# NoSameRain/RayTracingRenderer

Measured on AMD Instinct MI355X. Metric: Mray/s (traced closest-hit + shadow rays) at 1024x1024x64spp, synthetic 1M triangles, higher is better.
Workload: dtype f32; 1 GPU; C3: synth-1M, 1024x1024, 64 spp, MAX_DEPTH 4; triangles=1000000, width=1024, height=1024, spp=64, chunk_spp=64, max_depth=4, parallelism=one GPU, every tile (no exchange)

## Files before the change

### raytracingrenderer_amd/build.py

```python
import os
import shutil
import subprocess
import tempfile
import sys

ROOT = os.path.dirname(os.path.dirname(os.path.abspath(__file__)))
PKG = os.path.join(ROOT, "raytracingrenderer_amd")
CSRC = os.path.join(PKG, "csrc")
LIB = os.path.join(PKG, "lib")
ORACLE = os.path.join(ROOT, "oracle")
ORACLE_BUILD = os.path.join(ORACLE, "_build")
HIPCC = os.environ.get("HIPCC", "/opt/rocm/bin/hipcc")
ARCH = os.environ.get("RTG_ARCH", "gfx950")

HOST_SRC = ["host/image_io.cpp", "host/jpeg_decode.cpp", "host/gem_json.cpp", "host/scene_front.cpp"]
DEVICE_SRC = ["device/rtg_trace.hip", "device/rtg_scene.hip", "device/rtg_render.hip", "device/rtg_api.hip",
              "device/rtg_shade.hip", "device/rtg_light.hip", "device/rtg_multi.hip", "device/rtg_bvh.hip",
              "device/rtg_denoise.hip", "device/rtg_env.hip", "device/rtg_light_pick.hip",
              "device/rtg_shade_phys.hip", "device/rtg_shade_mis.hip"]
DEVICE_FLAGS = {"device/rtg_shade.hip": ["-mllvm", "-amdgpu-sched-strategy=max-ilp", "-fno-slp-vectorize"]}
DEVICE_FLAGS.update({"device/rtg_%s.hip" % u: ["-fno-slp-vectorize"] for u in ("trace", "scene", "render", "api")})
DEVICE_FLAGS["device/rtg_light_pick.hip"] = DEVICE_FLAGS["device/rtg_shade.hip"]
DEVICE_FLAGS["device/rtg_shade_phys.hip"] = DEVICE_FLAGS["device/rtg_shade.hip"]
DEVICE_FLAGS["device/rtg_shade_mis.hip"] = DEVICE_FLAGS["device/rtg_shade.hip"]
# ... 94 lines not shown

def build_device(force=False, debug=False):
    d = os.path.join(LIB, "debug") if debug else LIB
    os.makedirs(d, exist_ok=True)
    out = os.path.join(d, "librtg.so")
    if force or _stale(out, "device", "rtg-build-id:", debug):
        _compile_and_link(out, source_hash("device", debug), ["-DRTG_DEBUG=1"] if debug else [])
    return out


def build_variant(name, extra_flags):
    os.makedirs(os.path.join(LIB, "ab"), exist_ok=True)
    return _compile_and_link(os.path.join(LIB, "ab", name + ".so"), "ab-" + name, extra_flags)


def build_cli(force=False):
    out = os.path.join(LIB, "rtg_render")
    src = [os.path.join(CSRC, "host", "cli.cpp")]
    if not os.path.exists(src[0]):
        return None
    if force or _newer(out, _deps(src) + [os.path.join(LIB, "librth.so")]):
        _run(["g++", "-std=c++17", "-O2", "-ffp-contract=off", "-o", out] + src +
             ["-L" + LIB, "-lrth", "-lrtg", "-Wl,-rpath,$ORIGIN", "-ldl"])
    return out


def build_oracle(force=False):
    os.makedirs(ORACLE_BUILD, exist_ok=True)
    src = os.path.join(ORACLE, "rt_oracle.c")
    outs = []
    for flavour, libm in (("rtm", "0"), ("libm", "1")):
        out = os.path.join(ORACLE_BUILD, "liboracle_%s.so" % flavour)
        if force or _newer(out, _deps([src])):
            _run(["gcc", "-std=c11", "-O2", "-ffp-contract=off", "-fPIC", "-shared", "-D_GNU_SOURCE",
                  "-DORACLE_LIBM=" + libm, "-o", out, src, "-lm", "-lpthread"])
        outs.append(out)
    chk = os.path.join(ORACLE_BUILD, "libm_check")
    chk_src = os.path.join(ORACLE, "libm_check.c")
    if force or _newer(chk, _deps([chk_src])):
        _run(["gcc", "-std=c11", "-O2", "-ffp-contract=off", "-fno-builtin", "-pthread", "-o", chk, chk_src, "-lm"])
    outs.append(chk)
    dv = os.path.join(ORACLE_BUILD, "div_rewrites")
    dv_src = os.path.join(ORACLE, "div_rewrites.c")
    if force or _newer(dv, [dv_src]):
        _run(["gcc", "-std=c11", "-O2", "-ffp-contract=off", "-D_GNU_SOURCE", "-pthread", "-o", dv, dv_src, "-lm"])
    outs.append(dv)
    return outs


SAN_FLAGS = ["-O1", "-g", "-fsanitize=address,undefined", "-fno-sanitize-recover=all", "-fno-omit-frame-pointer",
             "-ffp-contract=off"]


def build_sanitized(force=False):
    nat = os.path.join(ROOT, "tests", "native")
    out_dir = os.path.join(nat, "_build")
    os.makedirs(out_dir, exist_ok=True)
    out = os.path.join(out_dir, "host_sanitize")
    drv = os.path.join(nat, "host_sanitize.cpp")
    orc = os.path.join(ORACLE, "rt_oracle.c")
    src = [os.path.join(CSRC, s) for s in HOST_SRC]
    if force or _newer(out, _deps(src + [drv, orc])):
        obj = os.path.join(out_dir, "rt_oracle_san.o")
        _run(["gcc", "-std=c11", "-D_GNU_SOURCE", "-DORACLE_LIBM=0", "-c", "-o", obj, orc] + SAN_FLAGS)
        _run(["g++", "-std=c++17", "-o", out, drv] + src + [obj] + SAN_FLAGS + ["-lz", "-lpthread", "-lm"])
    return out


def _build_test_program(name, extra_src, libs, force):
    nat = os.path.join(ROOT, "tests", "native")
    os.makedirs(os.path.join(nat, "_build"), exist_ok=True)
    out = os.path.join(nat, "_build", name)
    src = [os.path.join(nat, name + ".cpp")] + extra_src
    if force or _newer(out, _deps(src) + [os.path.join(LIB, "lib%s.so" % l) for l in libs]):
        _run([HIPCC, "-O2", "-std=c++17", "-ffp-contract=off", "-o", out] + src +
             ["-L" + LIB] + ["-l" + l for l in libs] + ["-Wl,-rpath," + LIB])
    return out


def build_sbvh_check(force=False):
    return _build_test_program("sbvh_check", [os.path.join(CSRC, "device", "rtg_bvh.hip")], ["rth"], force)


def build_scene_digest(force=False):
    return _build_test_program("scene_digest", [], ["rth", "rtg"], force)


def build_ref(force=False):
    mk = os.path.join(ORACLE, "ref", "Makefile")
    if not os.path.isdir("/root/reference/RTBase") or not os.path.exists(mk):
        return None
    _run(["make", "-s", "-C", os.path.join(ORACLE, "ref")] + (["-B"] if force else []))
    return os.path.join(ORACLE, "_ref", "libref.so")


def stage_assets():
    src = "/root/reference/RTBase"
    dst = os.path.join(ROOT, "assets")
    if not os.path.isdir(src):
        return
    os.makedirs(dst, exist_ok=True)
    for name in ("coffee", "bathroom", "materialball"):
        if os.path.isdir(os.path.join(src, name)) and not os.path.isdir(os.path.join(dst, name)):
            shutil.copytree(os.path.join(src, name), os.path.join(dst, name))
    for f, into in (("GI.hdr", ""), ("GI.hdr", "coffee")):
        d = os.path.join(dst, into, f)
        if os.path.exists(os.path.join(src, f)) and os.path.isdir(os.path.dirname(d)) and not os.path.exists(d):
            shutil.copy(os.path.join(src, f), d)


def build_all(force=False, device=True):
    stage_assets()
    build_host(force)
    if device:
        build_device(force)
        build_device(force, debug=True)
    build_cli(force)
    build_oracle(force)
    build_ref(force)


if __name__ == "__main__":
    build_all(force="--force" in sys.argv, device="--no-device" not in sys.argv)
    print("ok")
```

### raytracingrenderer_amd/csrc/device/rtg_bvh.hip

```cpp
#include "rtg_internal.h"

#include <algorithm>
#include <array>
#include <atomic>
#include <cmath>
#include <cstring>
#include <thread>
#include <vector>

namespace {

struct Ref {
    int tri;
    double lo[3], hi[3];
};

struct Box {
    double lo[3] = {INFINITY, INFINITY, INFINITY}, hi[3] = {-INFINITY, -INFINITY, -INFINITY};
    void add(const double* l, const double* h) {
        for (int a = 0; a < 3; ++a) { lo[a] = std::min(lo[a], l[a]); hi[a] = std::max(hi[a], h[a]); }
    }
    void add(const Ref& r) { add(r.lo, r.hi); }
    void add(const Box& b) { add(b.lo, b.hi); }
    bool empty() const { return lo[0] > hi[0]; }
    double area() const {
        if (empty()) return 0.0;
        const double x = hi[0] - lo[0], y = hi[1] - lo[1], z = hi[2] - lo[2];
        return x * y + y * z + z * x;
    }
};

double overlap_area(const Box& a, const Box& b) {
    Box o;
    for (int k = 0; k < 3; ++k) {
        o.lo[k] = std::max(a.lo[k], b.lo[k]);
        o.hi[k] = std::min(a.hi[k], b.hi[k]);
        if (o.lo[k] > o.hi[k]) return 0.0;
    }
    return o.area();
}

bool clip_bounds(const double v[3][3], const double* lo, const double* hi, double* out_lo, double* out_hi) {
    double a[12][3], b[12][3];
    int n = 3;
    for (int i = 0; i < 3; ++i)
        for (int k = 0; k < 3; ++k) a[i][k] = v[i][k];
    for (int ax = 0; ax < 3; ++ax)
        for (int side = 0; side < 2; ++side) {
            const double c = side ? hi[ax] : lo[ax];
            auto inside = [&](const double* p) { return side ? p[ax] <= c : p[ax] >= c; };
            int m = 0;
            for (int i = 0; i < n; ++i) {
                const double* p = a[i];
                const double* q = a[(i + 1) % n];
                const bool pi = inside(p), qi = inside(q);
                if (pi) { std::memcpy(b[m++], p, sizeof(double) * 3); }
                if (pi != qi && m < 12) {
                    const double t = (c - p[ax]) / (q[ax] - p[ax]);
                    for (int k = 0; k < 3; ++k) b[m][k] = p[k] + t * (q[k] - p[k]);
                    b[m][ax] = c;
                    ++m;
                }
            }
            n = std::min(m, 9);
            if (n == 0) return false;
            std::memcpy(a, b, sizeof(double) * 3 * n);
        }
    for (int k = 0; k < 3; ++k) { out_lo[k] = INFINITY; out_hi[k] = -INFINITY; }
    for (int i = 0; i < n; ++i)
        for (int k = 0; k < 3; ++k) {
            out_lo[k] = std::min(out_lo[k], a[i][k]);
            out_hi[k] = std::max(out_hi[k], a[i][k]);
        }
    for (int k = 0; k < 3; ++k) {
        out_lo[k] = std::max(out_lo[k], lo[k]);
        out_hi[k] = std::min(out_hi[k], hi[k]);
        if (out_lo[k] > out_hi[k]) return false;
    }
    return true;
}

struct Builder {
    const rtg_scene_desc* d;
    std::vector<int32_t> lk;
    std::vector<Ref> leaf_ref;
    double root_area = 0.0;
    long budget = 0;
// ... 139 lines not shown
        double best = INFINITY;
        ax = -1;
        for (int a = 0; a < 3; ++a)
            if (cost[a] < best) { best = cost[a]; ax = a; plane = pl[a]; }
        return best;
    }

    int build(std::vector<Ref>& r, int depth) {
        const int node = new_node();
        if (!ok) return node;
        if (depth > 120) { ok = false; return node; }
        if (depth >= stop_depth && r.size() > 1) {
            deferred.emplace_back(node, std::move(r));
            return node;
        }
        if (r.size() == 1) {
            leaf_ref[node] = r[0];
            lk[(size_t)node * 4 + 2] = r[0].tri;
            lk[(size_t)node * 4 + 3] = r[0].tri + 1;
            return node;
        }
        Box nb, cb;
        for (const Ref& x : r) {
            nb.add(x);
            double c[3];
            for (int k = 0; k < 3; ++k) c[k] = 0.5 * (x.lo[k] + x.hi[k]);
            cb.add(c, c);
        }
        std::vector<int> order;
        size_t cut = 0;
        Box bl, br;
        const double co = object_split(r, cb, order, cut, bl, br);
        const bool have_o = !order.empty() && cut > 0 && cut < r.size();
        int sax = -1;
        double plane = 0.0;
        double cs = INFINITY;
        if (budget > 0 && (!have_o || overlap_area(bl, br) > RTG_SBVH_ALPHA * root_area))
            cs = spatial_split(r, nb, sax, plane);
        std::vector<Ref> L, R;
        if (sax >= 0 && cs < co) {
            long dup = 0;
            for (const Ref& x : r) {
                if (x.hi[sax] <= plane) { L.push_back(x); continue; }
                if (x.lo[sax] >= plane) { R.push_back(x); continue; }
                double v[3][3];
                tri(x.tri, v);
                Ref a = x, b = x;
                double sl[3], sh[3];
                for (int k = 0; k < 3; ++k) { sl[k] = x.lo[k]; sh[k] = x.hi[k]; }
                sh[sax] = plane;
                const bool ka = clip_bounds(v, sl, sh, a.lo, a.hi);
                for (int k = 0; k < 3; ++k) { sl[k] = x.lo[k]; sh[k] = x.hi[k]; }
                sl[sax] = plane;
                const bool kb = clip_bounds(v, sl, sh, b.lo, b.hi);
                if (ka) L.push_back(a);
                if (kb) R.push_back(b);
                if (!ka && !kb) L.push_back(x);
                if (ka && kb) ++dup;
            }
            if (L.empty() || R.empty() || (L.size() >= r.size() && R.size() >= r.size())) {
                L.clear();
                R.clear();
            } else {
                budget -= dup;
            }
        }
        if (L.empty()) {
            if (have_o) {
                for (size_t i = 0; i < order.size(); ++i) (i < cut ? L : R).push_back(r[order[i]]);
            } else {
                L.assign(r.begin(), r.begin() + r.size() / 2);
                R.assign(r.begin() + r.size() / 2, r.end());
            }
        }
        std::vector<Ref>().swap(r);
        const int l = build(L, depth + 1);
        const int rr = build(R, depth + 1);
        lk[(size_t)node * 4] = l;
        lk[(size_t)node * 4 + 1] = rr;
        return node;
    }
};

}

bool build_sbvh(const rtg_scene_desc* d, std::vector<int32_t>& lk, std::vector<float>& bd) {
    const uint32_t nt = d->n_tris;
    if (nt < 2) return false;
    for (size_t k = 0; k < (size_t)nt * 9; ++k)
        if (!std::isfinite(d->positions[k])) return false;
    float scale = 0.0f;
    for (int k = 0; k < 6; ++k)
        if (std::isfinite(d->node_bounds[k])) scale = std::max(scale, std::fabs(d->node_bounds[k]));
    const double eta = std::ldexp((double)scale, -17);
    std::vector<Ref> refs(nt);
    Box root;
    for (uint32_t t = 0; t < nt; ++t) {
        const float* P = d->positions + (size_t)t * 9;
        refs[t].tri = (int)t;
        for (int k = 0; k < 3; ++k) {
            refs[t].lo[k] = std::min(std::min((double)P[k], (double)P[3 + k]), (double)P[6 + k]);
            refs[t].hi[k] = std::max(std::max((double)P[k], (double)P[3 + k]), (double)P[6 + k]);
        }
        root.add(refs[t]);
    }
    const int threads = (int)std::max(1u, std::min(16u, std::thread::hardware_concurrency()));
    Builder top(d);
    top.root_area = root.area();
    top.budget = (long)((double)nt * RTG_SBVH_DUP);
    top.stop_depth = nt < 50000 || threads == 1 ? (1 << 30) : 6;
    top.build(refs, 0);
    if (!top.ok) return false;
    const size_t nsub = top.deferred.size();
    std::vector<Builder> sub;
    sub.reserve(nsub);
    long deferred_refs = 0;
    for (auto& dr : top.deferred) deferred_refs += (long)dr.second.size();
    for (size_t k = 0; k < nsub; ++k) {
        sub.emplace_back(d);
        sub[k].root_area = top.root_area;
        sub[k].budget = deferred_refs ? (long)((double)top.budget * (double)top.deferred[k].second.size() / deferred_refs) : 0;
    }
    {
        std::atomic<size_t> next{0};
        std::vector<std::thread> pool;
        for (int t = 0; t < std::min<int>(threads, (int)nsub); ++t)
            pool.emplace_back([&]() {
                for (size_t k; (k = next.fetch_add(1)) < nsub;) sub[k].build(top.deferred[k].second, 6);
            });
        for (auto& t : pool) t.join();
    }
    for (const Builder& b : sub)
        if (!b.ok) return false;
    std::vector<int32_t> L = std::move(top.lk);
    std::vector<Ref> R = std::move(top.leaf_ref);
    for (size_t k = 0; k < nsub; ++k) {
        const int ph = top.deferred[k].first;
        const int base = (int)R.size();
        auto id = [&](int j) { return j == 0 ? ph : base + j - 1; };
        const Builder& b = sub[k];
        for (size_t j = 0; j < b.leaf_ref.size(); ++j) {
            int32_t w[4] = {b.lk[j * 4], b.lk[j * 4 + 1], b.lk[j * 4 + 2], b.lk[j * 4 + 3]};
            if (w[0] >= 0) { w[0] = id(w[0]); w[1] = id(w[1]); }
            if (j == 0) {
                std::memcpy(&L[(size_t)ph * 4], w, sizeof(w));
                R[ph] = b.leaf_ref[0];
            } else {
                L.insert(L.end(), w, w + 4);
                R.push_back(b.leaf_ref[j]);
            }
        }
    }
    const size_t nn = R.size();
    bd.assign(nn * 6, 0.0f);
    for (size_t i = nn; i-- > 0;) {
        float* o = &bd[i * 6];
        const Ref& x = R[i];
        if (L[i * 4] < 0) {
            for (int k = 0; k < 3; ++k) {
                o[k] = std::nextafter((float)(x.lo[k] - eta), -INFINITY);
                o[3 + k] = std::nextafter((float)(x.hi[k] + eta), INFINITY);
            }
        } else {
            const float* a = &bd[(size_t)L[i * 4] * 6];
            const float* b = &bd[(size_t)L[i * 4 + 1] * 6];
            for (int k = 0; k < 3; ++k) {
                o[k] = std::min(a[k], b[k]);
                o[3 + k] = std::max(a[3 + k], b[3 + k]);
            }
        }
    }
    lk = std::move(L);
    return true;
}
```

### raytracingrenderer_amd/csrc/device/rtg_internal.h

```cpp
#pragma once
#include "rtg_dev.h"
#include "../../../include/rtg.h"
#include "rtg_phys.h"
#include "rtg_mis.h"

#include <hip/hip_runtime.h>
#include <rocprofiler-sdk-roctx/roctx.h>

#include <string>
#include <vector>

using namespace rtgd;

#define RTG_TB 256
#define RTG_NSTATS 24
#ifndef RTG_TTB
#define RTG_TTB 64
#endif
#define RTG_POP ((int)0x80000001)
#ifndef RTG_STACK
#define RTG_STACK 16
#endif
#ifndef RTG_STACK_SMALL
#define RTG_STACK_SMALL 7
#endif
#ifndef RTG_SMALL_F4
#define RTG_SMALL_F4 192
#endif
#ifndef RTG_POSTPONE
#define RTG_POSTPONE 32
#endif
#ifndef RTG_MEM_PCT
#define RTG_MEM_PCT 50
#endif
#ifndef RTG_REFILL
#define RTG_REFILL 12
#endif
#ifndef RTG_TRACE_WPE
#define RTG_TRACE_WPE 7
#endif
#define RTG_CULL_REL 1.52587890625e-05f
#ifndef RTG_FETCH
#define RTG_FETCH 256
#endif
#ifndef RTG_FETCH_TAIL
#define RTG_FETCH_TAIL 8
#endif
#ifndef RTG_TAIL_BATCH
#define RTG_TAIL_BATCH 64
#endif
#ifndef RTG_LDS_MATS
#define RTG_LDS_MATS 64
#endif
#ifndef RTG_LDS_LIGHTS
#define RTG_LDS_LIGHTS 48
#endif
#ifndef RTG_LDS_PHYS
#define RTG_LDS_PHYS 64
#endif
#ifndef RTG_SHADE_WAVES
#define RTG_SHADE_WAVES 7
#endif
#ifndef RTG_SHADE_ENV_ALT_WAVES
#define RTG_SHADE_ENV_ALT_WAVES 4
#endif
#ifndef RTG_SAH_SWEEP
#define RTG_SAH_SWEEP 2048
#endif
#ifndef RTG_SAH_BINS
#define RTG_SAH_BINS 128
#endif
#ifndef RTG_SBVH_BINS
#define RTG_SBVH_BINS 32
#endif
#ifndef RTG_SBVH_ALPHA
#define RTG_SBVH_ALPHA 1e-5
#endif
#ifndef RTG_SBVH_DUP
#define RTG_SBVH_DUP 0.5
#endif
#define RTG_CAP_LEN 64
#ifndef RTG_DEBUG
#define RTG_DEBUG 0
#endif
#define RTG_CAM_PER_SAMPLE 1
#define RTG_CAM_LENS 2

#define RTG_CPAD(f) unsigned f; unsigned f##_pad[31];
struct __align__(16) Counters {
    RTG_CPAD(n_ext) RTG_CPAD(n_shadow) RTG_CPAD(f_ext) RTG_CPAD(f_shadow) RTG_CPAD(f_shade)
    RTG_CPAD(n_cam)
    RTG_CPAD(pad1) RTG_CPAD(pad2)
    unsigned f8[8 * 32];
    unsigned ne8[8 * 32];
    unsigned ns8[8 * 32];
};
#undef RTG_CPAD
static inline size_t seg_tiles(size_t P) { return ((P + 255) / 256 + 7) / 8; }
static inline size_t queue_slots(size_t P) { return seg_tiles(P) * 8 * 256; }

struct TraceIO {
    const unsigned* queue;
    const float4* ray_o;
    const float4* ray_d;
    const unsigned* count;
    float4* hits;
    const unsigned* squeue;
    const float4* sray_o;
    const float4* sray_d;
    const float4* sray_c;
    int spos;
    const unsigned* scount;
    float4* contrib;
    int* visible;
    unsigned* fetch;
    unsigned* fetch8;
    unsigned seg_cap;
    const unsigned* seg_ne;
    const unsigned* seg_ns;
    int* ovf;
    unsigned long long* stats;
    int cull;
    int wide;
    unsigned long long* wtime;
    uint4* cap;
    unsigned* cap_len;
    unsigned cap_n;
    float4 cam_o;
    unsigned* hcnt;
};

struct ChunkArgs {
    const unsigned* pixlist;
    unsigned npix, ns, s0, P;
    unsigned long long seed;
    int max_depth;
    int mode;
    DevCamera cam;
    int lean = 0;
    unsigned seg_tiles = 0;
    int cam_mode = 0;
    unsigned long long ns_mul = 0;
    unsigned ns_shift = 0;
};
static inline void set_ns_div(ChunkArgs& a) {
    a.ns_mul = 0;
    if ((unsigned long long)a.P > (1ull << 31)) return;
    unsigned l = 0;
    while ((1u << l) < a.ns) ++l;
    const unsigned S = 31 + l;
    a.ns_mul = ((1ull << S) + a.ns - 1) / a.ns;
    a.ns_shift = S;
}
static __device__ __forceinline__ void split_pid(const ChunkArgs& a, unsigned pid, unsigned& lp, unsigned& sl) {
    lp = a.ns_mul ? (unsigned)(((unsigned long long)pid * a.ns_mul) >> a.ns_shift) : pid / a.ns;
    sl = pid - lp * a.ns;
}

struct PathBufs {
    float4* thr;
    unsigned long long* rng;
    float4* ray_o;
// ... 121 lines not shown
    unsigned next_slot = 0;
    hipEvent_t entry = nullptr;
    hipEvent_t last_fold = nullptr;
    bool inflight = false;
    uint32_t pend_first = 0, pend_n = 0;
    uint64_t pend_seed = 0;
    std::vector<uint32_t> pend_key;
    int no_coalesce = 0;
    unsigned* d_pix = nullptr;
    size_t cap_pix = 0;
    std::vector<uint32_t> pix_key;
    unsigned npix = 0;
    unsigned* d_qctr = nullptr;
    unsigned long long* d_stats = nullptr;
    rtg_stats stats{};
    hipEvent_t ev[4] = {nullptr, nullptr, nullptr, nullptr};
    std::vector<hipEvent_t> kev;
    unsigned* h_cnt = nullptr;
    unsigned* d_hcnt = nullptr;
    int cap_cnt = 0;
    std::vector<hipEvent_t> tev;
    DenoiseState* dn = nullptr;
    int env_mode = RTG_ENV_UNIFORM;
    bool env_light = false;
    bool env_built = false;
    uint4* d_env_table = nullptr;
    std::vector<uint32_t> env_entries;
    std::vector<double> env_weights;
    double env_build_ms = 0.0;
    rtg_light_sampling light_sampling{RTG_LIGHTS_UNIFORM, 0.125f};
    bool light_built = false;
    float light_built_share = 0.0f;
    uint4* d_light_table = nullptr;
    std::vector<uint32_t> light_entries;
    std::vector<double> light_weights;
    double light_build_ms = 0.0;
    int material_model = RTG_MATERIALS_REFERENCE;
    std::vector<uint32_t> tri_mat;
    uint32_t n_desc_mats = 0;
    std::vector<rtg_material_params> mat_params;
    bool phys_built = false;
    bool phys_any = false;
    PhysMat* d_phys = nullptr;
    unsigned* d_phys_index = nullptr;
    int n_phys = 0;
    std::vector<unsigned> phys_index;
    int path_mis = RTG_PATH_MIS_OFF;
    std::vector<int32_t> light_tri;
    std::vector<int32_t> light_of;
    uint2* d_mis_index = nullptr;
    PhysMat* d_mis_ref = nullptr;
    int n_mis_ref = 0;
};
#define RTG_CNT_PENDING 0xFFFFFFFFu

struct HostScene {
    std::vector<DevNode> nodes;
    std::vector<DevNodeQ> nodesq;
    std::vector<float4> leafbox;
    std::vector<float4> img;
    int img_tri = 0, img_lb = 0;
    std::vector<DevTri48> tris48;
    std::vector<DevShade> shade;
    std::vector<DevMat> mats;
    std::vector<DevLight> lights;
    std::vector<DevTex> texinfo;
    std::vector<float> texels;
    int n_lights = 0, env_tex = -1, env_off = 0, env_w = 1, env_h = 1;
    bool env_uniform = false;
    float env_one[3] = {0.0f, 0.0f, 0.0f};
    int root_word = RTG_EXIT, root_wordw = RTG_EXIT;
    bool usew = false, rebuilt = false;
    uint32_t bvh_depth = 0, wide_depth = 0;
    float root_box[6] = {0, 0, 0, 0, 0, 0};
    float cull_scale = 0.0f;
    DevCamera cam{};
    rtg_camera_proj proj{};
    std::vector<uint32_t> tri_mat;
    uint32_t n_desc_mats = 0;
    std::vector<int32_t> light_tri;
};

bool build_sbvh(const rtg_scene_desc* d, std::vector<int32_t>& lk, std::vector<float>& bd);
int prepare_scene(const rtg_scene_desc* d, HostScene& hs);
int upload_scene(int device, const HostScene& hs, rtg_handle* h);
int size_trace_grids(rtg_handle* h);
static inline int trace_blocks_max(const rtg_handle* h) {
    return std::max({h->trace_blocks[0][0], h->trace_blocks[0][1], h->trace_blocks[1][0], h->trace_blocks[1][1]});
}
int capture_begin(rtg_handle* h, TraceIO& io, unsigned seg_tiles, hipStream_t ss);
int launch_trace(rtg_handle* h, const TraceIO& io, hipStream_t st, unsigned max_blocks = 0);
void free_chunk(ChunkSlot& sl);
int ensure_ovf(rtg_handle* h, ChunkSlot& sl);
int set_pixels(rtg_handle* h, const uint32_t* tiles, uint32_t n_tiles);
int ensure_chunk(rtg_handle* h, ChunkSlot& sl, size_t P, int maxb, bool queues);
int render_impl(rtg_handle* h, uint32_t first, uint32_t n_samples, uint64_t seed, const uint32_t* tiles,
                uint32_t n_tiles, hipStream_t st, bool lazy, bool add_spp = true);
int flush_pending(rtg_handle* h);
int join_frames(rtg_handle* h);
static inline CamSampling cam_sampling_dev(const rtg_handle* h) {
    const rtg_camera_sampling& c = h->cam_sampling;
    return CamSampling{c.filter, c.filter_radius, c.lens_radius, c.focal_distance};
}
static inline int cam_mode_of(const rtg_handle* h) {
    const rtg_camera_sampling& c = h->cam_sampling;
    if (c.filter == RTG_FILTER_NONE && !(c.lens_radius > 0.0f)) return 0;
    return RTG_CAM_PER_SAMPLE | (c.lens_radius > 0.0f ? RTG_CAM_LENS : 0);
}
int camera_sampling_check(const char* who, const rtg_camera_sampling* p);
int launch_generate(rtg_handle* h, const ChunkArgs& a, const PathBufs& pb, hipStream_t st);
int denoise_film(rtg_handle* h, const float* d_sum, uint32_t spp, const rtg_denoise_params* p, float* out);
int denoise_check_params(const char* who, const rtg_denoise_params* p);
void denoise_release(rtg_handle* h);
EnvTable env_table_of(const rtg_handle* h);
int env_cell_weights(rtg_handle* h, std::vector<double>& wts);
LightPick light_pick_of(const rtg_handle* h);
int light_sampling_check(const char* who, const rtg_light_sampling* p);
int launch_shade_pick(bool alt, bool tab, unsigned grid, hipStream_t st, const SceneView& s, const ChunkArgs& a,
                      const PathBufs& p, int b, const EnvTable& env, const LightPick& pick);
PhysArgs phys_args_of(const rtg_handle* h);
int launch_shade_phys(bool alt, bool tab, unsigned grid, hipStream_t st, const SceneView& s, const ChunkArgs& a,
                      const PathBufs& p, int b, const EnvTable& env, const LightPick& pick, const PhysArgs& phys);
int mis_sync_tables(rtg_handle* h);
bool path_mis_active(const rtg_handle* h);
int launch_shade_mis(const rtg_handle* h, bool tab, unsigned grid, hipStream_t st, const ChunkArgs& a, const PathBufs& p,
                     int b, const EnvTable& env, const LightPick& pick, const PhysArgs& phys);
int material_params_check(const char* who, const rtg_material_params* params, uint32_t n, uint32_t n_materials);
int launch_shade(bool alt, bool tab, unsigned grid, hipStream_t st, const SceneView& s, const ChunkArgs& a,
                 const PathBufs& p, int b, const EnvTable* env = nullptr);
```

### raytracingrenderer_amd/csrc/device/rtg_scene.hip

```cpp
#include "rtg_internal.h"

#include <algorithm>
#include <array>
#include <cmath>
#include <cstring>

static float host_bits_f(int v) { float f; std::memcpy(&f, &v, 4); return f; }

static bool encode_qnode(const float* bounds, const std::vector<int>& slots, const int32_t* words, DevNodeQ& out) {
    float lo[3], hi[3];
    for (int a = 0; a < 3; ++a) {
        lo[a] = bounds[(size_t)slots[0] * 6 + a];
        hi[a] = bounds[(size_t)slots[0] * 6 + 3 + a];
        for (int k = 1; k < (int)slots.size(); ++k) {
            lo[a] = std::min(lo[a], bounds[(size_t)slots[k] * 6 + a]);
            hi[a] = std::max(hi[a], bounds[(size_t)slots[k] * 6 + 3 + a]);
        }
    }
    unsigned planes[6] = {0, 0, 0, 0, 0, 0};
    unsigned bexp[3];
    for (int a = 0; a < 3; ++a) {
        const double ext = (double)hi[a] - (double)lo[a];
        int e = ext > 0 ? (int)std::ceil(std::log2(ext / 255.0)) : -126;
        e = std::max(e, -126);
// ... 201 lines not shown
        const float* U = d->uvs + (size_t)i * 6;
        if (d->material[i] >= d->n_materials) { g_err = "triangle material index out of range"; return RTG_ERR_ARG; }
        shade[i].a = make_float4(N[0], N[1], N[2], N[3]);
        shade[i].b = make_float4(N[4], N[5], N[6], N[7]);
        shade[i].c = make_float4(N[8], U[0], U[1], U[2]);
        shade[i].d = make_float4(U[3], U[4], U[5], host_bits_f((int)d->material[i]));
    }
    const uint32_t nn = d->n_nodes;
    if (nn == 0) { g_err = "BVH has no nodes"; return RTG_ERR_ARG; }
    std::vector<int> internal_id(nn, -1);
    int n_internal = 0;
    for (uint32_t i = 0; i < nn; ++i)
        if (d->node_links[i * 4 + 0] >= 0) internal_id[i] = n_internal++;
    auto word = [&](int node, int& out) -> bool {
        const int32_t* L = d->node_links + (size_t)node * 4;
        if (L[0] >= 0) { out = internal_id[node]; return true; }
        int cnt = L[3] - L[2];
        if (cnt < 1 || cnt > 2 || L[2] < 0 || (uint32_t)L[3] > nt) return false;
        out = ~(L[2] * RTG_LEAF_SPAN + (cnt - 1));
        return true;
    };
    std::vector<DevNode> nodes(std::max(n_internal, 1));
    uint32_t depth = 0;
    {
        std::vector<std::pair<int, uint32_t>> st{{0, 0}};
        while (!st.empty()) {
            auto [i, dep] = st.back();
            st.pop_back();
            depth = std::max(depth, dep);
            const int32_t* L = d->node_links + (size_t)i * 4;
            if (L[0] < 0) continue;
            if (L[0] >= (int)nn || L[1] < 0 || L[1] >= (int)nn) { g_err = "bad BVH link"; return RTG_ERR_ARG; }
            const float* bl = d->node_bounds + (size_t)L[0] * 6;
            const float* br = d->node_bounds + (size_t)L[1] * 6;
            DevNode& dn = nodes[internal_id[i]];
            dn.a = make_float4(bl[0], bl[1], bl[2], bl[3]);
            dn.b = make_float4(bl[4], bl[5], br[0], br[1]);
            dn.c = make_float4(br[2], br[3], br[4], br[5]);
            int wl, wr;
            if (!word(L[0], wl) || !word(L[1], wr)) {
                g_err = "BVH leaf with other than 1-2 triangles (MAXNODE_TRIANGLES = 2)";
                return RTG_ERR_ARG;
            }
            dn.d = make_int4(wl, wr, 0, 0);
            st.push_back({L[1], dep + 1});
            st.push_back({L[0], dep + 1});
        }
    }
    hs.bvh_depth = depth;
    int root_word = RTG_EXIT;
    if (nt > 0) {
        if (!word(0, root_word)) { g_err = "bad BVH root"; return RTG_ERR_ARG; }
    }
    std::vector<DevNodeQ> nodesq;
    bool qok = true;
    int root_wordw = root_word;
    bool finite = true;
    for (size_t k = 0; k < (size_t)nn * 6; ++k) finite = finite && std::isfinite(d->node_bounds[k]);
    for (uint32_t i = 0; finite && i < nn; ++i) {
        const int32_t* L = d->node_links + (size_t)i * 4;
        if (L[0] < 0) continue;
        const float* P = d->node_bounds + (size_t)i * 6;
        for (int c : {L[0], L[1]}) {
            const float* Cb = d->node_bounds + (size_t)c * 6;
            for (int q = 0; q < 3; ++q) finite = finite && Cb[q] >= P[q] && Cb[q + 3] <= P[q + 3];
        }
    }
    if (nt > 0 && finite && d->node_links[0] >= 0) {
        std::vector<int32_t> rlk;
        std::vector<float> rbd;
        const bool rebuilt = build_sbvh(d, rlk, rbd) || rebuild_over_leaves(d, rlk, rbd);
        const int32_t* LK = rebuilt ? rlk.data() : d->node_links;
        const float* BD = rebuilt ? rbd.data() : d->node_bounds;
        const uint32_t nn = rebuilt ? (uint32_t)(rlk.size() / 4) : d->n_nodes;
        auto wordw = [&](int node, int& out) -> bool {
            const int32_t* L = LK + (size_t)node * 4;
            const int cnt = L[3] - L[2];
            if (L[0] >= 0 || cnt < 1 || cnt > 2 || L[2] < 0 || (uint32_t)L[3] > nt) return false;
            out = ~(L[2] * RTG_LEAF_SPAN + (cnt - 1));
            return true;
        };
        hs.rebuilt = rebuilt;
        auto internal = [&](int i) { return LK[(size_t)i * 4] >= 0; };
        auto area = [&](int i) {
            const float* b = BD + (size_t)i * 6;
            const double x = b[3] - b[0], y = b[4] - b[1], z = b[5] - b[2];
            return x * y + y * z + z * x;
        };
        auto cut = [&](int n2) {
            std::vector<int> slots;
            slots = {LK[(size_t)n2 * 4], LK[(size_t)n2 * 4 + 1]};
            while ((int)slots.size() < 4) {
                int best_k = -1;
                for (int k = 0; k < (int)slots.size(); ++k)
                    if (internal(slots[k]) && (best_k < 0 || area(slots[k]) > area(slots[best_k]))) best_k = k;
                if (best_k < 0) break;
                const int c = slots[best_k];
                slots[best_k] = LK[(size_t)c * 4];
                slots.push_back(LK[(size_t)c * 4 + 1]);
            }
            return slots;
        };
        nodesq.emplace_back();
        root_wordw = 0;
        std::vector<std::array<int, 3>> work{{0, 0, 1}};
        while (!work.empty()) {
            auto [n2, nw, lvl] = work.back();
            work.pop_back();
            hs.wide_depth = std::max(hs.wide_depth, (uint32_t)lvl);
            const std::vector<int> slots = cut(n2);
            int32_t wq[4] = {RTG_EXIT, RTG_EXIT, RTG_EXIT, RTG_EXIT};
            for (int k = 0; k < (int)slots.size(); ++k) {
                if (internal(slots[k])) {
                    wq[k] = (int)nodesq.size();
                    nodesq.emplace_back();
                    work.push_back({slots[k], wq[k], lvl + 1});
                } else if (!wordw(slots[k], wq[k])) {
                    g_err = "bad BVH leaf";
                    return RTG_ERR_ARG;
                }
            }
            if (!encode_qnode(BD, slots, wq, nodesq[nw])) { qok = false; break; }
        }
    }
    float cull_scale = 0.0f;
    for (int k = 0; k < 6; ++k)
        if (std::isfinite(d->node_bounds[k])) cull_scale = std::max(cull_scale, std::fabs(d->node_bounds[k]));
    hs.usew = finite && qok && nt > 0 && cull_scale >= 0x1p-60f && cull_scale <= 0x1p60f;
    std::vector<float4> leafbox(std::max<size_t>((size_t)nt * 2, 2));
    for (uint32_t i = 0; i < nn; ++i) {
        const int32_t* L = d->node_links + (size_t)i * 4;
        if (L[0] >= 0) continue;
        const float* b = d->node_bounds + (size_t)i * 6;
        for (int t = L[2]; t < L[3]; ++t) {
            leafbox[2 * (size_t)t] = make_float4(b[0], b[1], b[2], b[3]);
            leafbox[2 * (size_t)t + 1] = make_float4(b[4], b[5], 0.0f, 0.0f);
        }
    }
    const bool small = hs.usew && nodesq.size() * 4 + (size_t)nt * 3 <= RTG_SMALL_F4;
    if (small) {
        hs.img.clear();
        for (const DevNodeQ& q : nodesq) hs.img.insert(hs.img.end(), q.q, q.q + 4);
        hs.img_tri = (int)hs.img.size();
        for (const DevTri48& t : tris48) hs.img.insert(hs.img.end(), {t.a, t.b, t.c});
        hs.img_lb = (int)hs.img.size();
    }
    std::vector<DevMat> mats(d->n_materials);
    for (uint32_t i = 0; i < d->n_materials; ++i) {
        const rtg_material& m = d->materials[i];
        if (m.texture < 0 || (uint32_t)m.texture >= d->n_textures) { g_err = "material texture out of range"; return RTG_ERR_ARG; }
        mats[i].kind = m.kind;
        mats[i].two_sided = m.two_sided;
        mats[i].tex = m.texture;
        const float lm = ((0.2126f * m.emission[0]) + (0.7152f * m.emission[1])) + (0.0722f * m.emission[2]);
        mats[i].is_light = lm > 0 ? 1 : 0;
        mats[i].int_ior = m.int_ior;
        mats[i].ext_ior = m.ext_ior;
        mats[i].emission = make_float4(m.emission[0], m.emission[1], m.emission[2], 0.0f);
    }
    std::vector<DevTex> texinfo(d->n_textures);
    std::vector<float> texels;
    for (uint32_t i = 0; i < d->n_textures; ++i) {
        const rtg_texture& t = d->textures[i];
        if (t.width <= 0 || t.height <= 0 || !t.texels) { g_err = "empty texture"; return RTG_ERR_ARG; }
        texinfo[i] = DevTex{(int)(texels.size() / 4), t.width, t.height, 0};
        for (size_t j = 0; j < (size_t)t.width * t.height; ++j)
            texels.insert(texels.end(), {t.texels[3 * j], t.texels[3 * j + 1], t.texels[3 * j + 2], 0.0f});
    }
    if (d->env_texture >= (int)d->n_textures) { g_err = "env texture out of range"; return RTG_ERR_ARG; }
    std::vector<char> uniform_tex(d->n_textures, 1);
    for (uint32_t i = 0; i < d->n_textures; ++i) {
        const rtg_texture& t = d->textures[i];
        const size_t n = (size_t)t.width * t.height;
        for (size_t j = 1; j < n && uniform_tex[i]; ++j)
            uniform_tex[i] = std::memcmp(t.texels + 3 * j, t.texels, 3 * sizeof(float)) == 0;
    }
    for (uint32_t i = 0; i < d->n_materials; ++i) {
        const DevTex& t = texinfo[mats[i].tex];
        if (t.w > 0xffff || t.h > 0xffff) { g_err = "texture larger than 65535 texels per side"; return RTG_ERR_ARG; }
        mats[i].tex = t.off;
        mats[i].tex_wh = (int)((unsigned)t.w | ((unsigned)t.h << 16));
        mats[i].uniform = uniform_tex[(size_t)(&t - texinfo.data())] ? 1 : 0;
        mats[i].texel0 = make_float4(texels[(size_t)t.off * 4], texels[(size_t)t.off * 4 + 1], texels[(size_t)t.off * 4 + 2], 0.0f);
    }
// ... 66 lines not shown
```

Baseline: 3867 Mray/s.

## Optimise SBVH topology by SAH-driven subtree reinsertion after build

Adds a post-build BVH optimiser that repeatedly removes the children of high-cost internal nodes and reinserts them at the position of minimal SAH cost, using a branch-and-bound search. It runs first on each deferred subtree in parallel and then on the top level. The tree is then relaid out in depth-first order. The aim is to cut node visits per ray during traversal, at the cost of longer host build time. It also always defers subtrees when there are many triangles, and moves the wide-node cut into a shared helper.

```diff
diff --git a/raytracingrenderer_amd/build.py b/raytracingrenderer_amd/build.py
--- a/raytracingrenderer_amd/build.py
+++ b/raytracingrenderer_amd/build.py
@@ -200,6 +200,10 @@
     return _build_test_program("sbvh_check", [os.path.join(CSRC, "device", "rtg_bvh.hip")], ["rth"], force)
 
 
+def build_walk_model(force=False):
+    return _build_test_program("walk_model", [os.path.join(CSRC, "device", "rtg_bvh.hip")], ["rth"], force)
+
+
 def build_scene_digest(force=False):
     return _build_test_program("scene_digest", [], ["rth", "rtg"], force)
 
diff --git a/raytracingrenderer_amd/csrc/device/rtg_bvh.hip b/raytracingrenderer_amd/csrc/device/rtg_bvh.hip
--- a/raytracingrenderer_amd/csrc/device/rtg_bvh.hip
+++ b/raytracingrenderer_amd/csrc/device/rtg_bvh.hip
@@ -3,6 +3,7 @@
 #include <algorithm>
 #include <array>
 #include <atomic>
+#include <chrono>
 #include <cmath>
 #include <cstring>
 #include <thread>
@@ -308,9 +309,216 @@
     }
 };
 
+struct Optimiser {
+    std::vector<int32_t>& L;
+    const std::vector<Ref>& R;
+    std::vector<int> parent, height;
+    std::vector<Box> box;
+    std::vector<double> area;
+    std::vector<char> stop;
+
+    Optimiser(std::vector<int32_t>& l, const std::vector<Ref>& r)
+        : L(l), R(r), parent(r.size(), -1), height(r.size(), 0), box(r.size()), area(r.size(), 0.0), stop(r.size(), 0) {}
+
+    bool leaf(int n) const { return L[(size_t)n * 4] < 0 || stop[n]; }
+    int& child(int n, int k) { return L[(size_t)n * 4 + k]; }
+
+    void refit_one(int n) {
+        const int a = child(n, 0), b = child(n, 1);
+        box[n] = box[a];
+        box[n].add(box[b]);
+        area[n] = box[n].area();
+        height[n] = 1 + std::max(height[a], height[b]);
+    }
+    void refit_up(int n) {
+        for (; n >= 0; n = parent[n]) refit_one(n);
+    }
+    void replace_child(int g, int from, int to, int& root) {
+        parent[to] = g;
+        if (g < 0) { root = to; return; }
+        child(g, child(g, 0) == from ? 0 : 1) = to;
+    }
+    int unlink(int x, int& root) {
+        const int f = parent[x];
+        const int y = child(f, 0) == x ? child(f, 1) : child(f, 0);
+        const int g = parent[f];
+        replace_child(g, f, y, root);
+        refit_up(g);
+        return f;
+    }
+    void link(int x, int y, int f, int& root) {
+        replace_child(parent[y], y, f, root);
+        child(f, 0) = y;
+        child(f, 1) = x;
+        parent[y] = parent[x] = f;
+        refit_up(f);
+    }
+
+    struct Cand {
+        double cost;
+        int node, depth;
+        bool operator<(const Cand& o) const { return cost > o.cost || (cost == o.cost && node > o.node); }
+    };
+    int best_position(int x, int root, int limit, std::vector<Cand>& heap) const {
+        const Box& bx = box[x];
+        const double ax = area[x];
+        double best_cost = INFINITY;
+        int best = -1;
+        heap.clear();
+        heap.push_back(Cand{0.0, root, 0});
+        while (!heap.empty()) {
+            std::pop_heap(heap.begin(), heap.end());
+            const Cand c = heap.back();
+            heap.pop_back();
+            if (c.cost + ax >= best_cost) break;
+            Box u = box[c.node];
+            u.add(bx);
+            const double total = c.cost + u.area();
+            if (total < best_cost && c.depth + 1 + std::max(height[c.node], height[x]) <= limit) {
+                best_cost = total;
+                best = c.node;
+            }
+            const double below = total - area[c.node];
+            if (!leaf(c.node) && below + ax < best_cost)
+                for (int k = 0; k < 2; ++k) {
+                    heap.push_back(Cand{below, L[(size_t)c.node * 4 + k], c.depth + 1});
+                    std::push_heap(heap.begin(), heap.end());
+                }
+        }
+        return best;
+    }
+
+    void reinsert_children(int n, int& root, int limit, std::vector<Cand>& heap) {
+        int a = child(n, 0), b = child(n, 1);
+        if (area[a] < area[b]) std::swap(a, b);
+        const int s = child(parent[n], 0) == n ? child(parent[n], 1) : child(parent[n], 0);
+        const int f1 = unlink(a, root);
+        const int f2 = unlink(b, root);
+        const int pa = best_position(a, root, limit, heap);
+        if (pa >= 0) {
+            link(a, pa, f1, root);
+            const int pb = best_position(b, root, limit, heap);
+            if (pb >= 0) { link(b, pb, f2, root); return; }
+            unlink(a, root);
+        }
+        child(f1, 0) = a;
+        child(f1, 1) = b;
+        parent[a] = parent[b] = f1;
+        refit_one(f1);
+        link(f1, s, f2, root);
+    }
+
+    int region(int root, int limit, const SbvhOpt& o) {
+        std::vector<int> nodes, st{root};
+        while (!st.empty()) {
+            const int n = st.back();
+            st.pop_back();
+            nodes.push_back(n);
+            if (leaf(n)) continue;
+            for (int k = 0; k < 2; ++k) { parent[child(n, k)] = n; st.push_back(child(n, k)); }
+        }
+        parent[root] = -1;
+        for (size_t i = nodes.size(); i-- > 0;) {
+            const int n = nodes[i];
+            if (stop[n]) continue;
+            if (L[(size_t)n * 4] >= 0) { refit_one(n); continue; }
+            box[n] = Box();
+            box[n].add(R[n]);
+            area[n] = box[n].area();
+            height[n] = 0;
+        }
+        std::vector<std::pair<double, int>> rank;
+        std::vector<Cand> heap;
+        auto area_sum = [&] {
+            double s = 0.0;
+            for (int n : nodes)
+                if (!leaf(n)) s += area[n];
+            return s;
+        };
+        double before = area_sum();
+        for (int pass = 0; pass < o.passes; ++pass) {
+            rank.clear();
+            for (int n : nodes) {
+                if (leaf(n) || n == root) continue;
+                const double a = area[n], c0 = area[child(n, 0)], c1 = area[child(n, 1)];
+                double m = a;
+                if (o.priority == 0) {
+                    const double mean = 0.5 * (c0 + c1), mn = std::min(c0, c1);
+                    m = mean > 0.0 && mn > 0.0 ? a * (a / mean) * (a / mn) : (a > 0.0 ? INFINITY : 0.0);
+                }
+                rank.emplace_back(m, n);
+            }
+            if (rank.empty()) break;
+            std::sort(rank.begin(), rank.end(), [](const std::pair<double, int>& x, const std::pair<double, int>& y) {
+                return x.first > y.first || (x.first == y.first && x.second < y.second);
+            });
+            const size_t take = std::min(rank.size(), std::max<size_t>(1, (size_t)((double)rank.size() * o.frac)));
+            for (size_t i = 0; i < take; ++i) {
+                const int n = rank[i].second;
+                if (n != root) reinsert_children(n, root, limit, heap);
+            }
+            const double after = area_sum();
+            const bool done = before - after < o.stop * before;
+            before = after;
+            if (done) break;
+        }
+        return root;
+    }
+};
+
+void optimise_bvh2(std::vector<int32_t>& L, std::vector<Ref>& R, const std::vector<int>& sub_roots, size_t n_top,
+                   int threads, const SbvhOpt& o) {
+    Optimiser op(L, R);
+    std::vector<int> new_root(sub_roots.size());
+    {
+        std::atomic<size_t> next{0};
+        std::vector<std::thread> pool;
+        for (int t = 0; t < std::min<int>(threads, (int)sub_roots.size()); ++t)
+            pool.emplace_back([&]() {
+                for (size_t k; (k = next.fetch_add(1)) < sub_roots.size();) new_root[k] = op.region(sub_roots[k], 100, o);
+            });
+        for (auto& t : pool) t.join();
+    }
+    if (!sub_roots.empty()) {
+        std::vector<int> moved(R.size(), -1);
+        for (size_t k = 0; k < sub_roots.size(); ++k) {
+            moved[sub_roots[k]] = new_root[k];
+            op.stop[new_root[k]] = 1;
+        }
+        for (size_t i = 0; i < n_top; ++i)
+            if (L[i * 4] >= 0 && moved[i] < 0)
+                for (int k = 0; k < 2; ++k)
+                    if (moved[L[i * 4 + k]] >= 0) L[i * 4 + k] = moved[L[i * 4 + k]];
+    }
+    const int root = op.region(0, 120, o);
+    std::vector<int32_t> L2;
+    std::vector<Ref> R2;
+    L2.reserve(L.size());
+    R2.reserve(R.size());
+    std::vector<std::pair<int, int>> st{{root, -1}};
+    while (!st.empty()) {
+        const auto [n, slot] = st.back();
+        st.pop_back();
+        const int id = (int)R2.size();
+        if (slot >= 0) L2[slot] = id;
+        L2.insert(L2.end(), &L[(size_t)n * 4], &L[(size_t)n * 4] + 4);
+        R2.push_back(R[n]);
+        if (L[(size_t)n * 4] < 0) continue;
+        st.push_back({L[(size_t)n * 4 + 1], id * 4 + 1});
+        st.push_back({L[(size_t)n * 4], id * 4});
+    }
+    L.swap(L2);
+    R.swap(R2);
 }
 
+}
+
 bool build_sbvh(const rtg_scene_desc* d, std::vector<int32_t>& lk, std::vector<float>& bd) {
+    SbvhOpt opt;
+    return build_sbvh_opt(d, lk, bd, opt);
+}
+
+bool build_sbvh_opt(const rtg_scene_desc* d, std::vector<int32_t>& lk, std::vector<float>& bd, SbvhOpt& opt) {
     const uint32_t nt = d->n_tris;
     if (nt < 2) return false;
     for (size_t k = 0; k < (size_t)nt * 9; ++k)
@@ -334,7 +542,7 @@
     Builder top(d);
     top.root_area = root.area();
     top.budget = (long)((double)nt * RTG_SBVH_DUP);
-    top.stop_depth = nt < 50000 || threads == 1 ? (1 << 30) : 6;
+    top.stop_depth = nt < 50000 ? (1 << 30) : 6;
     top.build(refs, 0);
     if (!top.ok) return false;
     const size_t nsub = top.deferred.size();
@@ -358,6 +566,7 @@
     }
     for (const Builder& b : sub)
         if (!b.ok) return false;
+    const size_t n_top = top.leaf_ref.size();
     std::vector<int32_t> L = std::move(top.lk);
     std::vector<Ref> R = std::move(top.leaf_ref);
     for (size_t k = 0; k < nsub; ++k) {
@@ -377,6 +586,13 @@
             }
         }
     }
+    if (opt.passes > 0 && nt >= opt.min_tris) {
+        std::vector<int> sub_roots;
+        for (auto& dr : top.deferred) sub_roots.push_back(dr.first);
+        const auto t0 = std::chrono::steady_clock::now();
+        optimise_bvh2(L, R, sub_roots, n_top, threads, opt);
+        opt.ms = std::chrono::duration<double, std::milli>(std::chrono::steady_clock::now() - t0).count();
+    }
     const size_t nn = R.size();
     bd.assign(nn * 6, 0.0f);
     for (size_t i = nn; i-- > 0;) {
diff --git a/raytracingrenderer_amd/csrc/device/rtg_internal.h b/raytracingrenderer_amd/csrc/device/rtg_internal.h
--- a/raytracingrenderer_amd/csrc/device/rtg_internal.h
+++ b/raytracingrenderer_amd/csrc/device/rtg_internal.h
@@ -78,6 +78,21 @@
 #endif
 #ifndef RTG_SBVH_DUP
 #define RTG_SBVH_DUP 0.5
+#endif
+#ifndef RTG_BVH_OPT_PASSES
+#define RTG_BVH_OPT_PASSES 20
+#endif
+#ifndef RTG_BVH_OPT_FRAC
+#define RTG_BVH_OPT_FRAC 1.0
+#endif
+#ifndef RTG_BVH_OPT_PRIORITY
+#define RTG_BVH_OPT_PRIORITY 0
+#endif
+#ifndef RTG_BVH_OPT_STOP
+#define RTG_BVH_OPT_STOP 1e-5
+#endif
+#ifndef RTG_BVH_OPT_MIN_TRIS
+#define RTG_BVH_OPT_MIN_TRIS 50000
 #endif
 #define RTG_CAP_LEN 64
 #ifndef RTG_DEBUG
@@ -365,6 +380,36 @@
 };
 
 bool build_sbvh(const rtg_scene_desc* d, std::vector<int32_t>& lk, std::vector<float>& bd);
+struct SbvhOpt {
+    int passes = RTG_BVH_OPT_PASSES;
+    double frac = RTG_BVH_OPT_FRAC;
+    int priority = RTG_BVH_OPT_PRIORITY;
+    double stop = RTG_BVH_OPT_STOP;
+    uint32_t min_tris = RTG_BVH_OPT_MIN_TRIS;
+    double ms = 0.0;
+};
+bool build_sbvh_opt(const rtg_scene_desc* d, std::vector<int32_t>& lk, std::vector<float>& bd, SbvhOpt& opt);
+static inline int wide_cut(const int32_t* lk, const float* bd, int n2, int slots[4]) {
+    auto internal = [&](int i) { return lk[(size_t)i * 4] >= 0; };
+    auto area = [&](int i) {
+        const float* b = bd + (size_t)i * 6;
+        const double x = b[3] - b[0], y = b[4] - b[1], z = b[5] - b[2];
+        return x * y + y * z + z * x;
+    };
+    int n = 2;
+    slots[0] = lk[(size_t)n2 * 4];
+    slots[1] = lk[(size_t)n2 * 4 + 1];
+    while (n < 4) {
+        int best_k = -1;
+        for (int k = 0; k < n; ++k)
+            if (internal(slots[k]) && (best_k < 0 || area(slots[k]) > area(slots[best_k]))) best_k = k;
+        if (best_k < 0) break;
+        const int c = slots[best_k];
+        slots[best_k] = lk[(size_t)c * 4];
+        slots[n++] = lk[(size_t)c * 4 + 1];
+    }
+    return n;
+}
 int prepare_scene(const rtg_scene_desc* d, HostScene& hs);
 int upload_scene(int device, const HostScene& hs, rtg_handle* h);
 int size_trace_grids(rtg_handle* h);
diff --git a/raytracingrenderer_amd/csrc/device/rtg_scene.hip b/raytracingrenderer_amd/csrc/device/rtg_scene.hip
--- a/raytracingrenderer_amd/csrc/device/rtg_scene.hip
+++ b/raytracingrenderer_amd/csrc/device/rtg_scene.hip
@@ -307,24 +307,10 @@
         };
         hs.rebuilt = rebuilt;
         auto internal = [&](int i) { return LK[(size_t)i * 4] >= 0; };
-        auto area = [&](int i) {
-            const float* b = BD + (size_t)i * 6;
-            const double x = b[3] - b[0], y = b[4] - b[1], z = b[5] - b[2];
-            return x * y + y * z + z * x;
-        };
         auto cut = [&](int n2) {
-            std::vector<int> slots;
-            slots = {LK[(size_t)n2 * 4], LK[(size_t)n2 * 4 + 1]};
-            while ((int)slots.size() < 4) {
-                int best_k = -1;
-                for (int k = 0; k < (int)slots.size(); ++k)
-                    if (internal(slots[k]) && (best_k < 0 || area(slots[k]) > area(slots[best_k]))) best_k = k;
-                if (best_k < 0) break;
-                const int c = slots[best_k];
-                slots[best_k] = LK[(size_t)c * 4];
-                slots.push_back(LK[(size_t)c * 4 + 1]);
-            }
-            return slots;
+            int s[4];
+            const int n = wide_cut(LK, BD, n2, s);
+            return std::vector<int>(s, s + n);
         };
         nodesq.emplace_back();
         root_wordw = 0;
```

New measurement: 3934 Mray/s (median of 6 runs). 1.02x the previous value.
